# kolinko/effort

Measured on AMD Instinct MI355X. Metric: effective GB/s + tokens/s vs effort %, Mistral-7B FFN 4096x11008 fp16, higher is better.
Workload: dtype f16

## Files before the change

effort_amd/_lib.py:

```python
from __future__ import annotations

import ctypes as C
import os
import subprocess

_HERE = os.path.dirname(os.path.abspath(__file__))
LAB_LIB_PATH = os.path.join(_HERE, "libeffort_hip_lab.so")
LIB_PATH = (LAB_LIB_PATH if os.environ.get("EFFORT_HIP_LIB") == "lab" else os.environ.get("EFFORT_HIP_LIB")) or os.path.join(_HERE, "libeffort_hip.so")

ERRORS = {
    -1: "EFFORT_ERR_ARG", -2: "EFFORT_ERR_SHAPE", -3: "EFFORT_ERR_EFFORT", -4: "EFFORT_ERR_HIP",
    -5: "EFFORT_ERR_KIND", -6: "EFFORT_ERR_CONVERT", -7: "EFFORT_ERR_BLAS", -8: "EFFORT_ERR_COMM",
}


class EffortError(RuntimeError):
    def __init__(self, code: int, where: str, detail: str = ""):
        self.code = code
        super().__init__(f"{where}: {ERRORS.get(code, code)} {detail}".strip())


def build(verbose: bool = False) -> str:
    cmd = ["make", "-C", os.path.join(_HERE, "csrc"), "-j8", "all"]
    res = subprocess.run(cmd, capture_output=not verbose, text=True)
# ... 55 lines not shown
    "effort_convert_status": (C.c_int, [_P, C.POINTER(C.c_int)]),
    "effort_q4_outlier_count": (C.c_int64, [C.c_int, C.c_int, C.c_double]),
    "effort_convert_q4": (C.c_int, [_P, _P, C.c_int, C.c_int, C.c_double, _P, _P, _P, _P]),
    "effort_top2_softmax": (C.c_int, [_P, _P, C.c_int, _P, _P]),
    "effort_mix2": (C.c_int, [_P, _P, _P, _P, _P, C.c_int]),
    "effort_moe_route": (C.c_int, [_P, _P, _P, _P, C.c_int, C.c_int, _P, _P, _P]),
    "effort_mix2_add": (C.c_int, [_P, _P, _P, _P, _P, C.c_int]),
    "effort_dense_gemv": (C.c_int, [_P, _P, _P, _P, C.c_int, C.c_int]),
    "effort_dense_gemv_expert": (C.c_int, [_P, _P, _P, _P, _P, C.c_int, C.c_int, C.c_int]),
    "effort_set_dense_backend": (C.c_int, [_P, C.c_int]),
    "effort_last_dispatch_count": (C.c_int, [_P, C.POINTER(C.c_uint32)]),
    "effort_last_cutoff": (C.c_int, [_P, C.POINTER(C.c_float)]),
    "effort_calc_dispatch": (C.c_int, [_P, _P, _P, _P, C.c_double, _P, _P]),
    "effort_convert_fp16": (C.c_int, [_P, _P, C.c_int, C.c_int, _P, _P, _P]),
    "effort_convert_fp16_pitched": (C.c_int, [_P, _P, C.c_int, C.c_int, _P, C.c_int, _P, _P]),
    "effort_cosine": (C.c_int, [_P, _P, _P, C.c_int, C.POINTER(C.c_float)]),
    "effort_set_split_cutoff": (C.c_int, [_P, C.c_int]),
    "effort_set_tuning": (C.c_int, [_P, C.c_int, C.c_int, C.c_int]),
    "effort_is_lab_build": (C.c_int, []),
    "effort_enable_kernel_timing": (C.c_int, [_P, C.c_int]),
    "effort_debug_stamps": (C.c_int, [_P, C.POINTER(C.c_ulonglong)]),
    "effort_debug_slice_counts": (C.c_int, [_P, C.c_int, C.POINTER(C.c_uint32), C.c_int]),
    "effort_debug_plan": (C.c_int, [C.c_int, C.c_int, C.c_int, C.c_int, _P, _P, _P, _P, _P, _P, C.c_int, C.c_int, C.c_int, C.c_int, _P, _P, _P, _P, _P, _P, _P, _P, _P]),
    "effort_debug_lanes": (C.c_int, [C.c_int, C.c_int, _P, C.c_int64, _P]),
    "effort_debug_trace": (C.c_int, [_P, C.POINTER(C.c_ulonglong), C.c_int]),
    "effort_kernel_clock": (C.c_int, [_P, C.POINTER(C.c_double), C.POINTER(C.c_int)]),
    "effort_kernel_timing": (C.c_int, [_P, C.POINTER(C.c_double), C.POINTER(C.c_double), C.POINTER(C.c_double), C.POINTER(C.c_int)]),
}

_lib = None


def lib() -> C.CDLL:
    global _lib
    if _lib is None:
        if not os.path.exists(LIB_PATH):
            raise RuntimeError(
                f"{LIB_PATH} is missing: the HIP extension has not been built "
                "(run `python -c 'import __graft_entry__ as g; g.build()'` or `make -C effort_amd/csrc`). "
                "effort_amd has no CPU fallback.")
        import torch
        l = C.CDLL(LIB_PATH)
        for name, (res, args) in _SIGS.items():
            if (name.startswith("effort_debug_") or name == "effort_is_lab_build") and os.environ.get("EFFORT_HIP_LIB") and not hasattr(l, name):
                continue
            fn = getattr(l, name)
# ... 9 lines not shown
```

effort_amd/csrc/api.hip:

```cpp
#include <dlfcn.h>
#include <rccl/rccl.h>
#include <rocblas/rocblas.h>

#include <cstdio>
#include <cstring>
#include <map>
#include <mutex>
#include <new>
#include <vector>

#include "../../include/effort_hip.h"
#include "../../include/effort_hip_debug.h"
#include "effort_internal.h"
#include "lanes.h"
#include "plan.h"
#include "sample_device.h"

using namespace effort;

static constexpr size_t kStampBytes = (size_t)(kTraceOff + kTraceItems * 12) * 8;

struct Lane {
    hipStream_t own = nullptr;
    hipEvent_t done = nullptr;
    bool dirty = false;
    float* d_cutoff = nullptr;
    uint32_t* d_count = nullptr;
    float* d_slabs = nullptr;
    uint32_t* d_counters = nullptr;
    uint32_t* d_sliceCounts = nullptr;
    uint32_t* d_queue = nullptr;
    uint32_t lastCalls = 1, lastSliceOff[effort::kMaxGroup] = {0}, lastSlices[effort::kMaxGroup] = {0};
};

struct effort_ctx {
    static constexpr int kMaxLanes = effort::kMaxLanes;
    int device = 0;
    hipStream_t stream = nullptr;
    int numCU = 256;
    Lane lane[kMaxLanes];
    LaneBook book;
    int lastLane = 0;
    hipEvent_t forkEv = nullptr;
    size_t slabBytes = 0;
    uint32_t* d_blockScratch = nullptr;
    uint16_t* d_vhalf = nullptr;
    size_t vhalfElems = 0;
    float* d_cos = nullptr;
    uint16_t* d_convVals = nullptr;
    size_t convElems = 0;
    int* d_status = nullptr;
    int persistent = -1;
    static constexpr uint32_t kMaxTiles = 1024, kMaxSlices = 4096;
    static constexpr size_t kSlabBytes = (size_t)64 << 20;
    unsigned long long* d_tstamp = nullptr;
    double wallClockKHz = 100000.0;
    rocblas_handle blas = nullptr;
    ncclComm_t comm = nullptr;
    int commRank = 0, commWorld = 1;
    bool denseRocblas = false;
    int tuneW = 0, tuneE = 0, tuneS = 0;
    bool splitCutoff = false;
    bool rowReuse = false;
    bool timing = false;
    bool clock = false;
// ... 581 lines not shown
        ga.tstamp = c->clock ? c->d_tstamp : nullptr;
        ga.ablate = env.ablate; ga.trace = (c->clock && c->trace) ? 1u : 0u;
        ga.split = (c->splitCutoff ? 1u : 0u) | (lp.compact ? 4u : 0u) | (c->rowReuse ? 8u : 0u);
        ga.numCU = (uint32_t)c->numCU; ga.queue = L.d_queue;
        ga.count = lp.count; ga.totalTiles = lp.totalTiles; ga.totalItems = lp.totalItems;
        ga.persistent = lp.persistent; ga.cutJobs = lp.cutJobs; ga.staggerSleeps = lp.staggerSleeps;
        for (uint32_t k = 0; k < lp.count; k++) {
            const int i = (int)(lp.first + k);
            const effort_w* w = ws[i];
            const CallPlan& p = plan.call[i];
            CallDesc& a = ga.call[k];
            a.buckets = w->buckets; a.stats = lp.compact ? (const void*)w->means16 : w->stats; a.rankBound = w->rankBound; a.probes = w->probes; a.v = vs[i];
            a.expNo = expNos ? expNos[i] : nullptr; a.out = outs[i];
            a.ol = OutlierIndex{fmt == kQ4 ? w->olBlockPtr : nullptr, w->olEntry, w->olMeta};
            a.q = (uint16_t)(int)((double)(kProbes - 1) * (1.0 - efforts[i]));
            a.bucketsTrim = (uint16_t)w->viewTrim;
            a.pre = pc[i].pre; a.vAux = a.pre ? vAux[i] : nullptr; a.resid = resids ? resids[i] : nullptr;
            a.slabOff = p.slabOff; a.tileOff = (uint16_t)p.tileOff; a.sliceOff = (uint16_t)p.sliceOff; a.geom = (uint16_t)p.geom;
            ga.geom[p.geom] = p.g;
            ga.wgEnd8[k] = (uint16_t)p.itemEnd8;
            L.lastSliceOff[i] = p.sliceOff; L.lastSlices[i] = p.g.slices;
        }
        { const int frc = fork_lane(c, lc); if (frc != EFFORT_OK) return frc; }
        if (c->splitCutoff && !(env.ablate & 1u)) HIP_TRY(c, launch_find_cutoff_group(ga, st));
        HIP_TRY(c, launch_bucket_mul(fmt, plan.W, plan.E, ga, st));
    }
    L.lastCalls = (uint32_t)n;
    if (tm) { HIP_TRY(c, hipEventRecord(ev[1], st)); c->nSamples++; }
    return EFFORT_OK;
}

extern "C" int effort_bucketmul(effort_ctx* c, const effort_w* w, const float* v, const uint32_t* expNo, float* out, double effort) {
    return do_group(c, kFp16, 1, &w, &v, &expNo, &out, &effort);
}
extern "C" int effort_bucketmul_q4(effort_ctx* c, const effort_w* w, const float* v, const uint32_t* expNo, float* out, double effort) {
    return do_group(c, kQ4, 1, &w, &v, &expNo, &out, &effort);
}
extern "C" int effort_bucketmul_group(effort_ctx* c, int n, const effort_w* const* ws, const float* const* vs,
                                      const uint32_t* const* expNos, float* const* outs, const double* efforts) {
    return do_group(c, kFp16, n, ws, vs, expNos, outs, efforts);
}
extern "C" int effort_bucketmul_group_fused(effort_ctx* c, int n, const effort_w* const* ws, const float* const* vs,
                                            const uint32_t* const* expNos, float* const* outs, const double* efforts,
                                            const int* prologues, const void* const* vAux, const float* const* resids) {
    return do_group(c, kFp16, n, ws, vs, expNos, outs, efforts, prologues, vAux, resids);
}
// ... 31 lines not shown
    Lane& L = c->lane[c->lastLane];
    if (L.lastSlices[idx] == 0) {
        HIP_TRY(c, hipMemcpyAsync(host_out, L.d_count, 4, hipMemcpyDeviceToHost, c->stream));
        HIP_TRY(c, hipStreamSynchronize(c->stream));
        return EFFORT_OK;
    }
    static thread_local uint32_t h[effort_ctx::kMaxSlices];
    HIP_TRY(c, hipMemcpyAsync(h, L.d_sliceCounts + L.lastSliceOff[idx], (size_t)L.lastSlices[idx] * 4, hipMemcpyDeviceToHost, c->stream));
    HIP_TRY(c, hipStreamSynchronize(c->stream));
    uint32_t n = 0;
    for (uint32_t i = 0; i < L.lastSlices[idx]; i++) n += h[i];
    *host_out = n;
    return EFFORT_OK;
}
extern "C" int effort_debug_slice_counts(effort_ctx* c, int idx, uint32_t* host, int maxSlices) {
    if (!c || !host || idx < 0 || (uint32_t)idx >= c->lane[c->lastLane].lastCalls || maxSlices < 1) return EFFORT_ERR_ARG;
    { const int jrc = join_lanes(c); if (jrc != EFFORT_OK) return jrc; }
    Lane& L = c->lane[c->lastLane];
    const uint32_t n = L.lastSlices[idx] < (uint32_t)maxSlices ? L.lastSlices[idx] : (uint32_t)maxSlices;
    if (n) HIP_TRY(c, hipMemcpyAsync(host, L.d_sliceCounts + L.lastSliceOff[idx], (size_t)n * 4, hipMemcpyDeviceToHost, c->stream));
    HIP_TRY(c, hipStreamSynchronize(c->stream));
    return (int)n;
}
extern "C" int effort_debug_plan(int q4, int numCU, int lanes, int n, const int* inDim, const int* outDim, const int* percentLoad,
                                 const int* prologue, const int* hasResid, const double* effort, int persistent, int tuneW, int tuneE, int tuneS,
                                 int* we, int* slices, int* tiles, int* sliceRows, int* launchOf,
                                 int* launchPersistent, int* launchCutJobs, int* launchCompact, int* launchStagger) {
    if (numCU < 1 || lanes < 1 || lanes > effort_ctx::kMaxLanes || n < 1 || n > kMaxGroup || !inDim || !outDim || !effort || !we || !slices || !tiles ||
        !sliceRows || !launchOf || !launchPersistent || !launchCutJobs || !launchCompact || !launchStagger) return EFFORT_ERR_ARG;
    const Format fmt = q4 ? kQ4 : kFp16;
    effort_ctx c0;
    c0.numCU = numCU; c0.book.nLanes = lanes; c0.persistent = persistent; c0.tuneW = tuneW; c0.tuneE = tuneE; c0.tuneS = tuneS;
    c0.slabBytes = effort_ctx::kSlabBytes;
    PlanCall pc[kMaxGroup];
    for (int i = 0; i < n; i++) {
        const int load = q4 ? 8 : (percentLoad ? percentLoad[i] : 16);
        if (inDim[i] <= 0 || outDim[i] <= 0 || check_shape((uint32_t)inDim[i], (uint32_t)outDim[i]) != EFFORT_OK || load < 1 || load > 16) return EFFORT_ERR_SHAPE;
        if (!(effort[i] >= 0.0 && effort[i] <= 1.0)) return EFFORT_ERR_EFFORT;
        const uint32_t cols = (uint32_t)outDim[i] / (q4 ? 32u : 16u);
        pc[i] = PlanCall{(uint32_t)inDim[i], (uint32_t)outDim[i], cols, (uint32_t)load, cols * 2u, 1u, !q4, (uint16_t)(prologue ? prologue[i] : 0), hasResid && hasResid[i]};
    }
    GroupPlan plan;
    const int rc = plan_group(fmt, plan_env(&c0, lanes > 1, thin_effort(n, effort)), n, pc, &plan);
    if (rc != EFFORT_OK) return rc;
    we[0] = plan.W; we[1] = plan.E;
    for (int i = 0; i < n; i++) {
        const CallPlan& p = plan.call[i];
        slices[i] = (int)p.g.slices; tiles[i] = (int)p.g.tiles; sliceRows[i] = (int)p.g.sliceRows; launchOf[i] = (int)p.launch;
    }
    for (uint32_t l = 0; l < plan.nLaunches; l++) {
        const LaunchPlan& lp = plan.launch[l];
        launchPersistent[l] = (int)lp.persistent; launchCutJobs[l] = (int)lp.cutJobs; launchCompact[l] = lp.compact ? 1 : 0; launchStagger[l] = (int)lp.staggerSleeps;
    }
    return (int)plan.nLaunches;
}
extern "C" int effort_group_cutoff(effort_ctx* c, int idx, float* host_out) {
    if (!c || !host_out || idx < 0 || (uint32_t)idx >= c->lane[c->lastLane].lastCalls) return EFFORT_ERR_ARG;
    { const int jrc = join_lanes(c); if (jrc != EFFORT_OK) return jrc; }
    Lane& L = c->lane[c->lastLane];
    HIP_TRY(c, hipMemcpyAsync(host_out, L.d_cutoff + idx, 4, hipMemcpyDeviceToHost, c->stream));
    HIP_TRY(c, hipStreamSynchronize(c->stream));
    return EFFORT_OK;
}
extern "C" int effort_last_dispatch_count(effort_ctx* c, uint32_t* host_out) { return effort_group_dispatch_count(c, 0, host_out); }
extern "C" int effort_last_cutoff(effort_ctx* c, float* host_out) { return effort_group_cutoff(c, 0, host_out); }

extern "C" int effort_set_dense_backend(effort_ctx* c, int rocblas) {
    if (!c) return EFFORT_ERR_ARG;
    c->denseRocblas = rocblas != 0;
    return EFFORT_OK;
}
extern "C" int effort_dense_gemv(effort_ctx* c, const void* W, const float* v, float* out, int inDim, int outDim) {
    if (!c || !W || !v || !out || inDim <= 0 || outDim <= 0) return fail(c, EFFORT_ERR_ARG, "dense_gemv: bad argument");
    { const int jrc = join_lanes(c); if (jrc != EFFORT_OK) return jrc; }
    if (inDim % 16) return fail(c, EFFORT_ERR_SHAPE, "dense_gemv: inDim % 16 != 0 (helpers/mps.swift:18)");
    if (!c->denseRocblas && dense_gemv_supported((uint32_t)inDim, (uint32_t)outDim)) {
        HIP_TRY(c, launch_dense_gemv(static_cast<const uint16_t*>(W), v, out, (uint32_t)inDim, (uint32_t)outDim, c->stream));
        return EFFORT_OK;
// ... 301 lines not shown
```

effort_amd/csrc/bucket_mul.hip:

```cpp
#include <cstring>
#include <type_traits>

#include "cutoff_device.h"

namespace effort {

constexpr int kBatch = 16;
template <int E> __host__ __device__ constexpr int batch_rows() { return E >= 4 ? 8 : kBatch; }
constexpr int kRounds = 16;

#ifndef EFFORT_ABLATE_NOSCATTER
#define EFFORT_ABLATE_NOSCATTER 0
#endif
#ifndef EFFORT_ABLATE_NOLOAD
#define EFFORT_ABLATE_NOLOAD 0
#endif

constexpr int kMinWavesPerEU = 4;

#ifndef EFFORT_ROW_AUX
#define EFFORT_ROW_AUX 2
#endif
constexpr int kRowAux = EFFORT_ROW_AUX;
#define GA_PERSISTENT(ga) (PERSIST ? (ga).persistent : 0u)
// ... 163 lines not shown
        }
    } else
#pragma unroll
    for (int rr = 0; rr < kRounds; rr++) {
        if ((uint32_t)(rr * NT) + wave * 64u >= nSlots) continue;
        const uint32_t c = rr * NT + tid;
        uint32_t voff;
        if (FMT == kFp16) {
            const uint32_t rank = c >> lg, jl = c & mask;
            const bool ok = rank < rowsPerIn && jl < nb;
            voff = (rowBase + (ok ? rank * inDim + j0 + jl : j0)) * 8u + 4u;
        } else {
            voff = ((rowBase + j0 * 8u + (c < nSlots ? c : 0u)) * 2u + 1u) * 4u;
        }
        lds_dma_dword(rs, voff, ldsM + ((uint32_t)(rr * NT) + wave * 64u) * 4u);
    }
#pragma unroll
    for (int u = 0; u < (FMT == kFp16 ? 1 : 2); u++) {
        if ((uint32_t)(u * NT) + wave * 64u >= nb) continue;
        lds_dma_dword(rv, (j0 + (uint32_t)(u * NT + tid)) * 4u, ldsV + ((uint32_t)(u * NT) + wave * 64u) * 4u);
    }
}

template <int FMT, int E, int W, bool FUSED, bool COMPACT, bool PERSIST, typename Prefetch>
__device__ __forceinline__ void mul_item(const GroupKArgs& ga, const uint32_t item, const ItemRef& ref, char* smem, const LdsPlan& lp, uint32_t& cachedCall,
                                         float& cachedCutoff, const uint32_t par, const bool staged, const bool firstItem, Prefetch prefetch) {
    constexpr int NACC = Fmt<FMT>::kAcc;
    constexpr int TILE_F = NACC * E * 64;
    constexpr int TILE_L = Fmt<FMT>::kSlots * E * 64;
    constexpr int NT = 64 * W;
    constexpr int VPT = 4096 / NT;
    constexpr int KB = batch_rows<E>();

    const uint32_t ci = __builtin_amdgcn_readfirstlane(ref.ci), s = __builtin_amdgcn_readfirstlane(ref.s), t = __builtin_amdgcn_readfirstlane(ref.t);
    const CallDesc& a = ga.call[ci];
    const MulGeom& g = ga.geom[a.geom];
    float* const a_slabs = ga.slabs + (size_t)a.slabOff * 64u;
    uint32_t* const a_counters = ga.counters + a.tileOff;
    uint32_t* const a_sliceCounts = ga.sliceCounts + a.sliceOff;
    float* const a_cutoff = ga.cutoff + ci;
    (void)item;

    int tid0 = threadIdx.x;
    asm volatile("" : "+v"(tid0));
    const int tid = tid0, lane = tid & 63;
#ifdef EFFORT_CUT_FINE
    const bool wstamp = false;
#else
    const bool wstamp = GA_TSTAMP(ga) && tid == 0;
#endif
    unsigned long long ph[6] = {0, 0, 0, 0, 0, 0};
    if (wstamp) ph[0] = wall_clock64();
#ifdef EFFORT_CUT_FINE
    const bool stampCut = GA_TSTAMP(ga) && item == 0 && tid == 0, stamp = false;
#define EFFORT_PSTAMP(i) if (stampCut) GA_TSTAMP(ga)[26 + (i)] = clock64();
#else
#define EFFORT_PSTAMP(i)
// ... 286 lines not shown
            before[rr] = wtot;
            const uint32_t c = rr * NT + tid;
            bool k;
            if (FMT == kFp16) k = (cutoff < (kCutoffScale * half_bits_to_float((uint16_t)(mraw[u] >> 16))) * ax) & ((c >> lg) < g.rowsPerIn) & sel;
            else k = (cutoff < (kCutoffScale * __uint_as_float(mraw[u])) * fabsf(vq[u])) & (c < nSlots) & sel;
            keepMask |= k ? (1u << rr) : 0u;
            wtot += (uint32_t)__popcll(__ballot(k));
        }
    }
    uint32_t wbase = 0;
    if (lane == 0) wbase = atomicAdd(&flags[4], wtot);
    wbase = __builtin_amdgcn_readfirstlane(wbase);
#pragma unroll
    for (int rr = 0; rr < kRounds; rr++) {
        if ((uint32_t)(rr * NT) >= nSlots) break;
        const uint32_t c = rr * NT + tid;
        const bool k = (keepMask >> rr) & 1u;
        const unsigned long long m = __ballot(k);
        const uint32_t pos = wbase + before[rr] + __builtin_amdgcn_mbcnt_hi((uint32_t)(m >> 32), __builtin_amdgcn_mbcnt_lo((uint32_t)m, 0u));
        if (k) list[pos] = (uint16_t)(FMT == kFp16 ? (((c >> lg) << 12) | (c & ((1u << lg) - 1u))) : c);
    }
    __syncthreads();
    const uint32_t n = flags[4];
    const uint32_t code0 = list[(uint32_t)(wave * KB) + ((uint32_t)lane & (uint32_t)(KB - 1))];
    if (t == 0 && tid == 0) a_sliceCounts[s] = n;
    if (stamp) GA_TSTAMP(ga)[19] = wall_clock64();
    if (wstamp) ph[3] = wall_clock64();

    if constexpr (PERSIST) stream_geom();
    const bool colOK = vColOK != 0u;
    const __amdgpu_buffer_rsrc_t rsrc = __builtin_amdgcn_make_buffer_rsrc(
        reinterpret_cast<uint16_t*>((size_t)(uint32_t)__builtin_amdgcn_readfirstlane(vBuckLo) | ((size_t)(uint32_t)__builtin_amdgcn_readfirstlane(vBuckHi) << 32)), 0,
        (int)__builtin_amdgcn_readfirstlane(vRecords), 0x00020000);
    const uint32_t nU = (GA_ABLATE(ga) & 4u) ? 0u : __builtin_amdgcn_readfirstlane(n);
    uint32_t* const cursor = flags + 5;
    auto grab = [&]() -> uint32_t {
        uint32_t bq = 0;
        if (lane == 0) bq = atomicAdd(cursor, (uint32_t)KB);
        return __builtin_amdgcn_readfirstlane(bq);
    };

    auto decode_code = [&](uint32_t code, uint32_t& boff, float& dv) {
        {
            uint32_t rowIdx;
            if (FMT == kFp16) { const uint32_t rank = code >> 12, jl = code & 4095u; rowIdx = rank * vInDim + jl; dv = vblk[jl] * scale; }
            else {
                rowIdx = code;
                dv = __int_as_float(__float2int_rn((vblk[code >> 3] * means[code]) * scale));
            }
            boff = (vRow0 + rowIdx) * vRowPitch;
        }
    };
    auto decode = [&](uint32_t i0, uint32_t& boff, float& dv) {
// ... 119 lines not shown
            accumulate(pa, dvA, __builtin_amdgcn_readfirstlane(min((uint32_t)KB, nU - baseA)));
            if constexpr (OL) ol_add(entA);
            baseA = grab();
            decode(baseA, boffA, dvA);
            issue(aux, pa, boffA);
            if constexpr (OL) ol_fetch(entA);
            accumulate(pb, dvB, __builtin_amdgcn_readfirstlane(baseB < nU ? min((uint32_t)KB, nU - baseB) : 0u));
            if constexpr (OL) ol_add(entB);
        }
        if constexpr (OL) {
            while (olKa < olK1) {
                ol_fetch(entB); ol_add(entA);
                if (olKa >= olK1) break;
                ol_fetch(entA); ol_add(entB);
            }
        }
    };
    constexpr bool kRowSwitch = kRowAux != 0 && (PERSIST || E == 4);
    const bool rowsReused = kRowSwitch && (ga.split & 8u) != 0u;
    auto stream = [&](auto withOl) {
        if constexpr (kRowSwitch) { if (rowsReused) { stream_rows(withOl, std::integral_constant<int, 0>{}); return; } }
        stream_rows(withOl, std::integral_constant<int, kRowAux>{});
    };
    if constexpr (kOlMerge) { if (olEarly) stream(std::true_type{}); else stream(std::false_type{}); }
    else stream(std::false_type{});
    if (!asked) asked = prefetch();
    __syncthreads();
    if (stamp) GA_TSTAMP(ga)[20] = wall_clock64();
    if (wstamp) ph[4] = wall_clock64();

    float* const olsum = reinterpret_cast<float*>(smem + offM);
    if constexpr (FMT != kFp16) {
        if (olAny) {
            const OutlierIndex& ol = a.ol;
            float* const vfull = olEarly ? reinterpret_cast<float*>(smem + __builtin_amdgcn_readfirstlane(lp.offO)) : olsum + (olPer > kOlSumFloats ? olPer : kOlSumFloats);
            const bool vLds = g.inDim <= kOlLdsFloats;
            if constexpr (!kOlMerge) ol_share();
            const uint32_t bFirst = olBFirst, nB = olNB, parts = olParts;
            if (vLds && !olEarly) {
                for (uint32_t i0 = 0; i0 < g.inDim; i0 += NT * 8u) {
                    float x[8];
#pragma unroll
                    for (int u = 0; u < 8; u++) x[u] = a.v[min(i0 + u * NT + tid, g.inDim - 1u)];
                    if constexpr (FUSED) {
                        uint32_t xa[8];
#pragma unroll
// ... 123 lines not shown
            rec[1] = (unsigned long long)(__builtin_amdgcn_s_getreg((31 << 11) | 20) & 0xFu) | ((unsigned long long)(ci & 0xFu) << 4) | ((unsigned long long)(n & 0xFFFFu) << 8) | ((unsigned long long)(t & 0xFFu) << 24) |
                     ((unsigned long long)__builtin_amdgcn_s_getreg((31 << 11) | 4) << 32);
#pragma unroll
            for (int i = 0; i < 6; i++) rec[2 + i] = ph[i];
        }
        unsigned long long* line = GA_TSTAMP(ga) + 64 + (item & 31u) * 8u;
#pragma unroll
        for (int i = 0; i < 5; i++) atomicAdd(&line[i], ph[i + 1] - ph[i]);
        atomicAdd(&line[5], 1ull);
        atomicMin(&GA_TSTAMP(ga)[0], ph[0]);
        atomicMax(&GA_TSTAMP(ga)[26], ph[0]);
        atomicMax(&GA_TSTAMP(ga)[28], ph[5] - ph[0]);
        atomicMax(&GA_TSTAMP(ga)[29], ph[4] - ph[3]);
        atomicMax(&GA_TSTAMP(ga)[1], (unsigned long long)wall_clock64());
#endif
    };
    {
        __syncthreads();
        if (tid == 0) {
            const uint32_t ticket = __hip_atomic_fetch_add(&a_counters[t], 1u, __ATOMIC_RELAXED, __HIP_MEMORY_SCOPE_AGENT);
            flags[0] = (ticket == nSlices - 1u) ? 1u : 0u;
        }
        __syncthreads();
        if (flags[0] == 0u) { flush_stamps(); return; }
    }
    if (GA_ABLATE(ga) & 2u) { if (tid == 0) __hip_atomic_store(&a_counters[t], 0u, __ATOMIC_RELAXED, __HIP_MEMORY_SCOPE_AGENT); return; }

    const bool rstamp = GA_TSTAMP(ga) && ci == 0 && t == 0 && tid == 0;
    if (rstamp) GA_TSTAMP(ga)[23] = wall_clock64();
    typedef uint32_t u4v __attribute__((ext_vector_type(4)));
    const uint32_t sliceStride = __builtin_amdgcn_readfirstlane(vSliceStride);
    constexpr int kCols4 = TILE_F / 4;
    constexpr int G = NT / kCols4 >= 2 ? NT / kCols4 : 1;
    float* const gpart = reinterpret_cast<float*>(smem + offA + (uint32_t)TILE_L * 4u);
    static_assert(G == 1 || (uint32_t)TILE_L * 4u + (uint32_t)G * TILE_F * 4u <= (cutoff_table_bytes(NT) > (uint32_t)TILE_L * 4u ? cutoff_table_bytes(NT) : (uint32_t)TILE_L * 4u),
                  "the thread groups' partial sums must fit behind the tile");
    auto reduce_tile = [&](auto kc) {
        constexpr int kRed = decltype(kc)::value;
        const int grp = G > 1 ? tid / kCols4 : 0;
        const uint32_t per = G > 1 ? ((nSlices + G - 1) / G + 3u) / 4u * 4u : nSlices;
        const uint32_t sl0 = (uint32_t)grp * per, sl1 = min(nSlices, sl0 + per);
        for (int o = (G > 1 ? tid % kCols4 : tid) * 4; o < TILE_F; o += (G > 1 ? kCols4 : NT) * 4) {
            const uint32_t vo = t * (uint32_t)(TILE_F * 4) + (uint32_t)o * 4u;
            float res[4] = {0.0f, 0.0f, 0.0f, 0.0f};
            if (FUSED && a.resid && (G == 1 || grp == 0)) {
#pragma unroll
                for (int h = 0; h < 4; h++) {
// ... 48 lines not shown
    if (nSlices <= 8u * G) reduce_tile(std::integral_constant<int, 8>{});
    else reduce_tile(std::integral_constant<int, 16>{});
    if (PERSIST && G > 1) __syncthreads();
    if (rstamp) GA_TSTAMP(ga)[24] = wall_clock64();
    if (tid == 0) {
        __hip_atomic_store(&a_counters[t], 0u, __ATOMIC_RELAXED, __HIP_MEMORY_SCOPE_AGENT);
#if !defined(EFFORT_CUT_FINE) && !defined(EFFORT_PRODUCT_ONLY)
        if (GA_TSTAMP(ga)) {
            flush_stamps();
            const uint32_t done = __hip_atomic_fetch_add(ga.groupDone, 1u, __ATOMIC_RELAXED, __HIP_MEMORY_SCOPE_AGENT);
            if (done == ga.totalTiles - 1u) {
                const unsigned long long t0 = __hip_atomic_load(&GA_TSTAMP(ga)[0], __ATOMIC_RELAXED, __HIP_MEMORY_SCOPE_AGENT);
                const unsigned long long t1 = __hip_atomic_load(&GA_TSTAMP(ga)[1], __ATOMIC_RELAXED, __HIP_MEMORY_SCOPE_AGENT);
                GA_TSTAMP(ga)[2] += t1 - t0; GA_TSTAMP(ga)[3] += 1;
                GA_TSTAMP(ga)[27] += __hip_atomic_load(&GA_TSTAMP(ga)[26], __ATOMIC_RELAXED, __HIP_MEMORY_SCOPE_AGENT) - t0;
                __hip_atomic_store(&GA_TSTAMP(ga)[26], 0ull, __ATOMIC_RELAXED, __HIP_MEMORY_SCOPE_AGENT);
                __hip_atomic_store(&GA_TSTAMP(ga)[0], ~0ull, __ATOMIC_RELAXED, __HIP_MEMORY_SCOPE_AGENT);
                __hip_atomic_store(&GA_TSTAMP(ga)[1], 0ull, __ATOMIC_RELAXED, __HIP_MEMORY_SCOPE_AGENT);
                __hip_atomic_store(ga.groupDone, 0u, __ATOMIC_RELAXED, __HIP_MEMORY_SCOPE_AGENT);
            }
        }
#endif
    }
}

template <int NT>
__device__ __forceinline__ void cutoff_job(const GroupKArgs& ga, uint32_t ci, char* smem) {
    constexpr int VPT = 4096 / NT;
    const CallDesc& a = ga.call[ci];
    int tid0 = threadIdx.x;
    asm volatile("" : "+v"(tid0));
    const int tid = tid0;
    const uint32_t e = a.expNo ? a.expNo[0] : 0u;
    const uint16_t* pr = a.probes + (size_t)e * kProbes;
    float vj[VPT]; uint16_t prj[VPT];
#pragma unroll
    for (int i = 0; i < VPT; i++) { vj[i] = a.v[tid + NT * i]; prj[i] = pr[tid + NT * i]; }
    [[maybe_unused]] constexpr bool PERSIST = true;
    const unsigned long long tj0 = (GA_TSTAMP(ga) && GA_TRACE(ga)) ? wall_clock64() : 0ull;
    const float cutoff = block_find_cutoff<NT>(vj, prj, a.q, smem + cutoff_table_bytes(NT), reinterpret_cast<uint32_t*>(smem), []() {}, nullptr);
    if (tid == 0 && GA_TSTAMP(ga) && GA_TRACE(ga)) {
        unsigned long long* rec = GA_TSTAMP(ga) + kTraceOff + (size_t)ci * 8u;
        rec[0] = (unsigned long long)ci | ((unsigned long long)blockIdx.x << 32) | (1ull << 63);
        rec[1] = (unsigned long long)__builtin_amdgcn_s_getreg((31 << 11) | 20) | ((unsigned long long)__builtin_amdgcn_s_getreg((31 << 11) | 4) << 32);
        rec[2] = tj0; rec[3] = wall_clock64();
    }
// ... 11 lines not shown
    __shared__ unsigned long long s_next;
#ifdef EFFORT_CUT_FINE
    if (GA_TSTAMP(ga) && blockIdx.x == 0 && threadIdx.x == 0) GA_TSTAMP(ga)[26] = clock64();
#endif
    if constexpr (!PERSIST) {
        const uint32_t* const kw = reinterpret_cast<const uint32_t*>(&ga);
        uint32_t touch[12];
#pragma unroll
        for (int i = 0; i < 12; i++) touch[i] = kw[i * 16];
#pragma unroll
        for (int i = 0; i < 12; i++) asm volatile("" :: "s"(touch[i]));
    }
#ifdef EFFORT_CUT_FINE
#define EFFORT_ESTAMP(i) if (GA_TSTAMP(ga) && blockIdx.x == 0 && threadIdx.x == 0) GA_TSTAMP(ga)[16 + (i)] = clock64();
#else
#define EFFORT_ESTAMP(i)
#endif
    EFFORT_ESTAMP(0)
    const uint32_t staggerSleeps = ga.staggerSleeps;
    if constexpr (PERSIST) {
        if (GA_PERSISTENT(ga) && staggerSleeps && blockIdx.x >= ga.numCU)
            for (uint32_t i = 0; i < staggerSleeps; i++) __builtin_amdgcn_s_sleep(32);
    }
    const uint32_t total = ga.totalItems + GA_CUTJOBS(ga);
    uint32_t cachedCall = 0xFFFFFFFFu; float cachedCutoff = 0.0f;
    const uint32_t x = blockIdx.x & 7u;
    uint32_t dry = 0;
    auto pull = [&]() -> uint32_t {
        uint32_t got = total;
        for (uint32_t tries = 0; tries < 8u && got >= total; tries++) {
            const uint32_t q = (x + tries) & 7u;
            if ((dry >> q) & 1u) continue;
            const uint32_t cand = __hip_atomic_fetch_add(&ga.queue[q * 16u], 1u, __ATOMIC_RELAXED, __HIP_MEMORY_SCOPE_AGENT) * 8u + q;
            if (cand < total) got = cand; else dry |= 1u << q;
            if (GA_ABLATE(ga) & 64u) break;
        }
        return got;
    };
    auto pull_sync = [&]() -> uint32_t {
        if (threadIdx.x == 0) s_item = pull();
        __syncthreads();
        const uint32_t it = __builtin_amdgcn_readfirstlane(s_item);
        __syncthreads();
        return it;
    };
    constexpr bool kPipe = !FUSED && FMT == kFp16;
    const LdsPlan lp = ga.lp;
    uint32_t par = 0;
    bool staged = false;
    uint32_t gen = 0;
    if (threadIdx.x == 0) __hip_atomic_store(&s_next, 0ull, __ATOMIC_RELAXED, __HIP_MEMORY_SCOPE_WORKGROUP);
    uint32_t item = GA_PERSISTENT(ga) ? pull_sync() : blockIdx.x;
    while (item < total) {
        if (item < GA_CUTJOBS(ga)) {
            if (item < ga.count) cutoff_job<64 * W>(ga, item, smem);
            item = GA_PERSISTENT(ga) ? pull_sync() : total;
            continue;
        }
        ItemRef ref;
        EFFORT_ESTAMP(1)
        if (!locate_item(ga, item - GA_CUTJOBS(ga), ref)) {
            item = GA_PERSISTENT(ga) ? pull_sync() : total;
            continue;
        }
        EFFORT_ESTAMP(2)
        gen++;
        bool stagedNext = false;
        auto prefetch = [&]() -> bool {
            if (!GA_PERSISTENT(ga)) return true;
            if (threadIdx.x == 0)
                __hip_atomic_store(&s_next, ((unsigned long long)gen << 32) | (unsigned long long)pull(), __ATOMIC_RELAXED, __HIP_MEMORY_SCOPE_WORKGROUP);
            const unsigned long long nx = __hip_atomic_load(&s_next, __ATOMIC_RELAXED, __HIP_MEMORY_SCOPE_WORKGROUP);
            if (__builtin_amdgcn_readfirstlane((uint32_t)(nx >> 32)) != gen) return false;
            const uint32_t next = __builtin_amdgcn_readfirstlane((uint32_t)nx);
            ItemRef nref;
            if (kPipe && !(GA_ABLATE(ga) & 128u) && next >= GA_CUTJOBS(ga) && next < total && locate_item(ga, next - GA_CUTJOBS(ga), nref)) {
                int tid0 = threadIdx.x;
                asm volatile("" : "+v"(tid0));
                stage_issue<FMT, W, COMPACT>(ga, nref, tid0, smem, lp, par ^ 1u);
                stagedNext = true;
            }
            return true;
        };
        const bool firstOwn = gen == 1u && (GA_ABLATE(ga) & 512u) != 0u;
        mul_item<FMT, E, W, FUSED, COMPACT, PERSIST>(ga, item - GA_CUTJOBS(ga), ref, smem, lp, cachedCall, cachedCutoff, par, staged, firstOwn, prefetch);
        item = GA_PERSISTENT(ga) ? __builtin_amdgcn_readfirstlane((uint32_t)__hip_atomic_load(&s_next, __ATOMIC_RELAXED, __HIP_MEMORY_SCOPE_WORKGROUP)) : total;
        staged = stagedNext;
        par ^= 1u;
    }
    if (GA_PERSISTENT(ga) && threadIdx.x == 0) {
        const uint32_t gone = __hip_atomic_fetch_add(&ga.queue[8 * 16], 1u, __ATOMIC_RELAXED, __HIP_MEMORY_SCOPE_AGENT);
        if (gone == gridDim.x - 1u) {
            for (int i = 0; i <= 8; i++) __hip_atomic_store(&ga.queue[i * 16], 0u, __ATOMIC_RELAXED, __HIP_MEMORY_SCOPE_AGENT);
            for (int i = 0; i < kMaxGroup; i++) __hip_atomic_store(&ga.queue[9 * 16 + i], 0u, __ATOMIC_RELAXED, __HIP_MEMORY_SCOPE_AGENT);
        }
    }
}

template <int FMT, int E, int W, typename F>
static hipError_t each_variant(F&& f) {
    hipError_t err = hipSuccess;
    auto one = [&](auto fu, auto co, auto pe) {
        constexpr bool FU = decltype(fu)::value, CO = decltype(co)::value, PE = decltype(pe)::value;
        if (err == hipSuccess) err = f(&bucket_mul_kernel<FMT, E, W, FU, CO, PE>, FU, CO, PE);
    };
    constexpr std::true_type T{}; constexpr std::false_type N{};
    one(N, N, T); one(T, N, T);
    if constexpr (FMT == kFp16) one(N, T, T);
// ... 101 lines not shown
```

effort_amd/csrc/plan.h:

```cpp
#pragma once
#include "effort_internal.h"

namespace effort {

constexpr int kMaxLaunches = kMaxGroup / kMaxGeoms + 1;

struct PlanEnv {
    int numCU = 256, nLanes = 1;
    bool laned = false;
    int persistent = -1;
    int tuneW = 0, tuneE = 0, tuneS = 0;
    bool splitCutoff = false, clock = false;
    uint32_t ablate = 0;
    bool noJobs = false, noCompact = false;
    size_t slabBytes = 0;
    uint32_t maxTiles = 0, maxSlices = 0;
    bool thinEffort = false;
    int tailCalls = 0, tailMult = 0;
};
struct PlanCall {
    uint32_t inDim, outDim, cols, rowsPerIn, rowPitch, numExperts;
    bool hasMeans16;
    uint16_t pre;
    bool hasResid;
};
struct CallPlan {
    MulGeom g;
    uint32_t mult;
    uint32_t launch, geom;
    uint32_t slabOff, tileOff, sliceOff;
    uint32_t itemEnd8;
};
struct LaunchPlan {
    uint32_t first, count;
    uint32_t persistent, cutJobs, staggerSleeps;
    bool compact;
    uint32_t totalItems, totalTiles, realItems;
};
struct GroupPlan {
    int W = 0, E = 0;
    int err = 0;
    const char* msg = "";
    uint32_t nLaunches = 0;
    CallPlan call[kMaxGroup];
    LaunchPlan launch[kMaxLaunches];
};

bool supported(int W, int E);
int plan_group(Format fmt, const PlanEnv& env, int n, const PlanCall* calls, GroupPlan* plan);

}
```

effort_amd/csrc/plan.hip:

```cpp
#include <cstring>

#include "../../include/effort_hip.h"
#include "plan.h"

namespace effort {

static uint32_t round8(uint32_t x) { return (x + 7u) / 8u * 8u; }
static uint32_t min_slices(uint32_t inDim) { return round8((inDim + 511u) / 512u); }
static uint32_t max_slices(uint32_t inDim) { return round8((inDim + 127u) / 128u); }
static uint32_t tiles_at(const PlanCall& w, int E) { return (w.cols + 64 * E - 1) / (64 * E); }
static uint32_t group_tiles(int n, const PlanCall* ws, int E) {
    uint32_t t = 0;
    for (int i = 0; i < n; i++) t += tiles_at(ws[i], E);
    return t;
}
static uint32_t padded_items(uint32_t tiles, uint32_t slices) { return round8(tiles * slices); }
static uint32_t padded_min_items(int n, const PlanCall* ws, int E) {
    uint32_t t = 0;
    for (int i = 0; i < n; i++) t += padded_items(tiles_at(ws[i], E), min_slices(ws[i].inDim));
    return t;
}
static bool fits_one_round(const PlanEnv& env, int n, uint32_t tiles, uint32_t allTiles, uint32_t s) {
    const bool same = allTiles == (uint32_t)n * tiles;
    return (same ? (uint32_t)n * padded_items(tiles, s) : allTiles * s + 7u * (uint32_t)n) <= (uint32_t)env.numCU;
// ... 153 lines not shown
static uint32_t geom_index(MulGeom* geoms, uint32_t& n, const MulGeom& g) {
    uint32_t k = 0;
    while (k < n && memcmp(&geoms[k], &g, sizeof(g)) != 0) k++;
    if (k == n && n < (uint32_t)kMaxGeoms) geoms[n++] = g;
    return k;
}

static void finish_launch(Format fmt, const PlanEnv& env, int W, const PlanCall* ws, const GroupPlan* P, LaunchPlan* lp) {
    const uint32_t R = env.persistent < 0 ? 2u : (uint32_t)env.persistent;
    const uint32_t perCU = (env.persistent < 0 && fmt == kFp16 && !env.laned) ? 6u : R;
    lp->persistent = (R && lp->realItems > (uint32_t)env.numCU * perCU) ? R : 0u;
    bool plain = true;
    for (uint32_t i = 0; i < lp->count; i++) plain = plain && !ws[lp->first + i].pre;
    lp->cutJobs = (lp->persistent && !env.splitCutoff && plain && !env.noJobs) ? (lp->count + 7u) / 8u * 8u : 0u;
    const bool leanGrid = lp->persistent == 0u && W == 8 && !env.clock && !env.ablate;
    bool compact = fmt == kFp16 && !env.noCompact && (leanGrid || (lp->persistent != 0u && plain));
    for (uint32_t i = 0; compact && !leanGrid && i < lp->count; i++) compact = !ws[lp->first + i].hasResid;
    for (uint32_t i = 0; compact && i < lp->count; i++) {
        const MulGeom& g = P->call[lp->first + i].g;
        compact = ws[lp->first + i].hasMeans16 && g.inDim % 2u == 0u && g.sliceRows % 2u == 0u;
    }
    lp->compact = compact;
    lp->staggerSleeps = (lp->persistent && fmt == kQ4 && !env.laned) ? 11u : 0u;
}

int plan_group(Format fmt, const PlanEnv& env, int n, const PlanCall* ws, GroupPlan* P) {
    P->err = EFFORT_OK; P->msg = ""; P->nLaunches = 0;
    const bool laned = env.laned;
    const int W = env.tuneW ? env.tuneW : 8;
    const int E = pick_elems(env, fmt, n, ws);
    P->W = W; P->E = E;
    const char* const noGeometry = "bucketmul: no launch geometry for this shape/tuning";
    if (!supported(W, E)) return plan_fail(P, EFFORT_ERR_ARG, noGeometry);
    const uint32_t groupTiles = group_tiles(n, ws, E);
    MulGeom g1[kMaxGroup], g2[kMaxGroup];
    uint32_t it1[kMaxGroup], base = 0;
    for (int i = 0; i < n; i++) {
        const int rc = choose_geom(env, fmt, ws[i], n, W, E, groupTiles, 1, &g1[i]);
        if (rc != EFFORT_OK) return plan_fail(P, rc, noGeometry);
        it1[i] = padded_items(g1[i].tiles, g1[i].slices);
        base += it1[i];
    }
    int thinFrom = n;
    if (E == 2 && n >= 8 && !laned && !env.tuneS && env.persistent < 0 && !env.thinEffort) {
        const uint32_t round = 2u * (uint32_t)env.numCU, over = base % round;
        if (base > round && over != 0u && over * 32u <= round * 7u && (fmt != kFp16 || base <= 6u * (uint32_t)env.numCU)) {
// ... 65 lines not shown
```

effort_amd/runtime.py:

```python
from __future__ import annotations

import ctypes as C

import torch

from . import _lib


class Gpu:
    def __init__(self, device: int | None = None):
        if not torch.cuda.is_available():
            raise RuntimeError("effort_amd needs an AMD GPU (torch.cuda.is_available() is False); there is no CPU fallback")
        self.device = torch.cuda.current_device() if device is None else int(device)
        self._lib = _lib.lib()
        with torch.cuda.device(self.device):
            stream = torch.cuda.current_stream(self.device).cuda_stream
            self.ctx = self._lib.effort_create(self.device, C.c_void_p(stream))
        self.has_comm = False
        self.dense_rocblas = False
        if not self.ctx:
            raise RuntimeError("effort_create failed: " + (self._lib.effort_last_error(None) or b"").decode())
        self._stream = stream

    def _bind_stream(self):
# ... 105 lines not shown
            self.check(k, "slice_counts")
        return list(buf[:k])

    def debug_trace(self, n: int = 4096):
        buf = (C.c_ulonglong * (12 * n))()
        self.check(self._lib.effort_debug_trace(self.ctx, buf, n), "debug_trace")
        return [tuple(buf[8 * i:8 * i + 8]) + tuple(buf[8 * n + 4 * i:8 * n + 4 * i + 4]) for i in range(n)]

    def kernel_timing(self):
        mul, cut, integ, n = C.c_double(), C.c_double(), C.c_double(), C.c_int()
        self.check(self._lib.effort_kernel_timing(self.ctx, C.byref(mul), C.byref(cut), C.byref(integ), C.byref(n)), "kernel_timing")
        return {"mul_us": mul.value, "cutoff_us": cut.value, "integrate_us": integ.value, "samples": n.value}

    def last_dispatch_count(self, idx: int = 0) -> int:
        n = C.c_uint32()
        self.check(self._lib.effort_group_dispatch_count(self.ctx, int(idx), C.byref(n)), "last_dispatch_count")
        return int(n.value)

    def last_cutoff(self, idx: int = 0) -> float:
        x = C.c_float()
        self.check(self._lib.effort_group_cutoff(self.ctx, int(idx), C.byref(x)), "last_cutoff")
        return float(x.value)

    def close(self):
        if getattr(self, "ctx", None):
            self._lib.effort_destroy(self.ctx)
            self.ctx = None

    def __del__(self):
        try:
            self.close()
        except Exception:
            pass


def plan(calls, *, q4: bool = False, numCU: int = 256, lanes: int = 1, persistent: int = -1, waves: int = 0, elems: int = 0, slices: int = 0) -> dict:
    n = len(calls)
    rows = [tuple(c) + (16, 0, 0)[len(c) - 3:] for c in calls]
    ints = lambda k: (C.c_int * n)(*[int(r[k]) for r in rows])
    out = [(C.c_int * max(n, 2))() for _ in range(9)]
    k = _lib.lib().effort_debug_plan(int(q4), numCU, lanes, n, ints(0), ints(1), ints(3), ints(4), ints(5), (C.c_double * n)(*[float(r[2]) for r in rows]),
                                     persistent, waves, elems, slices, *out)
    if k < 0:
        raise _lib.EffortError(k, "plan")
    we, per_call, per_launch = out[0], out[1:5], out[5:]
    res = {"W": we[0], "E": we[1]}
    res.update({name: list(a[:n]) for name, a in zip(("slices", "tiles", "sliceRows", "launch"), per_call)})
    res.update({name: list(a[:k]) for name, a in zip(("persistent", "cutJobs", "compact", "stagger"), per_launch)})
    return res


def lanes(ops, *, lanes: int = 4) -> list[dict]:
    kinds = {"launch": 0, "timed": 1, "join": 2}
    words = []
    for op in ops:
        kind, cap, busy, rd, wr = tuple(op) + (0, (), ())[len(op) - 2:]
        words += [kinds[kind], int(cap), int(bool(busy)), len(rd), len(wr)]
        for lo, hi in list(rd) + list(wr):
            words += [int(lo), int(hi)]
    n, W = len(ops), 18
    out = (C.c_int64 * max(n * W, 1))()
    k = _lib.lib().effort_debug_lanes(lanes, n, (C.c_int64 * max(len(words), 1))(*words), len(words), out)
    if k < 0:
        raise _lib.EffortError(k, "lanes")
    members = lambda mask: tuple(i for i in range(lanes) if mask >> i & 1)
    res = []
    for i in range(n):
        r = out[i * W:(i + 1) * W]
        res.append({"rc": r[0], "joined_first": bool(r[1]), "joined": members(r[2]), "lane": r[3], "fork_waited": bool(r[4]), "waits": members(r[5]),
                    "pending": members(r[6]), "nextLane": r[7], "busyStreak": r[8], "migrated": bool(r[9]),
                    "reads": list(r[10:10 + lanes]), "writes": list(r[14:14 + lanes])})
    return res
# ... 14 lines not shown
```

include/effort_hip_debug.h:

```cpp
#ifndef EFFORT_HIP_DEBUG_H
#define EFFORT_HIP_DEBUG_H

#include "effort_hip.h"

#ifdef __cplusplus
extern "C" {
#endif

EFFORT_API int effort_set_tuning(effort_ctx* ctx, int wavesPerGroup, int elemsPerLane, int rowSlices);
EFFORT_API int effort_set_split_cutoff(effort_ctx* ctx, int split);

EFFORT_API int effort_set_persistent(effort_ctx* ctx, int wgPerCU);

EFFORT_API int effort_debug_hook_lane(effort_ctx* ctx, int lane);

EFFORT_API int effort_is_lab_build(void);
EFFORT_API int effort_enable_kernel_timing(effort_ctx* ctx, int enable);
EFFORT_API int effort_kernel_clock(effort_ctx* ctx, double* mul_us_avg, int* n_launches);
EFFORT_API int effort_kernel_timing(effort_ctx* ctx, double* mul_us_avg, double* cutoff_us_avg,
                         double* integrate_us_avg, int* n_samples);
EFFORT_API int effort_debug_occupancy(effort_ctx* ctx, int q4, int waves, int elems, int ldsBytes);
EFFORT_API int effort_debug_stamps(effort_ctx* ctx, unsigned long long* host32);
EFFORT_API int effort_debug_slice_counts(effort_ctx* ctx, int idx, uint32_t* host, int maxSlices);
EFFORT_API int effort_debug_plan(int q4, int numCU, int lanes, int n, const int* inDim, const int* outDim, const int* percentLoad,
                      const int* prologue, const int* hasResid, const double* effort, int persistent, int tuneW, int tuneE, int tuneS,
                      int* we, int* slices, int* tiles, int* sliceRows, int* launchOf,
                      int* launchPersistent, int* launchCutJobs, int* launchCompact, int* launchStagger);
#define EFFORT_LANES_LAUNCH 0
#define EFFORT_LANES_TIMED 1
#define EFFORT_LANES_JOIN 2
#define EFFORT_LANES_OUT_WORDS 18
EFFORT_API int effort_debug_lanes(int lanes, int nOps, const int64_t* ops, int64_t nWords, int64_t* out);
EFFORT_API int effort_debug_trace(effort_ctx* ctx, unsigned long long* host, int maxRecords);

#ifdef __cplusplus
}
#endif
#endif
```

Before: 21490.

## Let persistent fp16 workgroups walk all tiles of a slice when lanes overlap

Adds a 'walk' mode for persistent compact fp16 launches. When other lanes are pending, each work unit is a (call, slice) pair, and the workgroup loops over every tile of that slice itself instead of pulling per-tile items. Slices are rotated per call to spread load. This is meant to cut work-queue traffic and per-item setup when the GPU is shared across concurrent lanes, at the cost of coarser load balancing and a more complex kernel loop. Debug entry points expose the unit count.

```diff
diff --git a/effort_amd/_lib.py b/effort_amd/_lib.py
--- a/effort_amd/_lib.py
+++ b/effort_amd/_lib.py
@@ -101,6 +101,8 @@
     "effort_debug_stamps": (C.c_int, [_P, C.POINTER(C.c_ulonglong)]),
     "effort_debug_slice_counts": (C.c_int, [_P, C.c_int, C.POINTER(C.c_uint32), C.c_int]),
     "effort_debug_plan": (C.c_int, [C.c_int, C.c_int, C.c_int, C.c_int, _P, _P, _P, _P, _P, _P, C.c_int, C.c_int, C.c_int, C.c_int, _P, _P, _P, _P, _P, _P, _P, _P, _P]),
+    "effort_debug_last_units": (C.c_int, [_P]),
+    "effort_debug_walk_units": (C.c_int, [C.c_int, C.c_int, C.c_int, C.c_int, _P, _P, _P, _P, _P, _P, C.c_int, C.c_int, C.c_int, C.c_int, C.c_int]),
     "effort_debug_lanes": (C.c_int, [C.c_int, C.c_int, _P, C.c_int64, _P]),
     "effort_debug_trace": (C.c_int, [_P, C.POINTER(C.c_ulonglong), C.c_int]),
     "effort_kernel_clock": (C.c_int, [_P, C.POINTER(C.c_double), C.POINTER(C.c_int)]),
diff --git a/effort_amd/csrc/api.hip b/effort_amd/csrc/api.hip
--- a/effort_amd/csrc/api.hip
+++ b/effort_amd/csrc/api.hip
@@ -41,6 +41,7 @@
     Lane lane[kMaxLanes];
     LaneBook book;
     int lastLane = 0;
+    uint32_t lastUnits = 0;
     hipEvent_t forkEv = nullptr;
     size_t slabBytes = 0;
     uint32_t* d_blockScratch = nullptr;
@@ -668,6 +669,8 @@
             L.lastSliceOff[i] = p.sliceOff; L.lastSlices[i] = p.g.slices;
         }
         { const int frc = fork_lane(c, lc); if (frc != EFFORT_OK) return frc; }
+        c->lastUnits = walk_units(plan, l, lc.laned, (c->book.pending_lanes() & ~(1u << lc.pick.lane)) != 0u);
+        if (c->lastUnits) ga.split |= 16u | (c->lastUnits / 8u) << 8;
         if (c->splitCutoff && !(env.ablate & 1u)) HIP_TRY(c, launch_find_cutoff_group(ga, st));
         HIP_TRY(c, launch_bucket_mul(fmt, plan.W, plan.E, ga, st));
     }
@@ -745,12 +748,9 @@
     HIP_TRY(c, hipStreamSynchronize(c->stream));
     return (int)n;
 }
-extern "C" int effort_debug_plan(int q4, int numCU, int lanes, int n, const int* inDim, const int* outDim, const int* percentLoad,
-                                 const int* prologue, const int* hasResid, const double* effort, int persistent, int tuneW, int tuneE, int tuneS,
-                                 int* we, int* slices, int* tiles, int* sliceRows, int* launchOf,
-                                 int* launchPersistent, int* launchCutJobs, int* launchCompact, int* launchStagger) {
-    if (numCU < 1 || lanes < 1 || lanes > effort_ctx::kMaxLanes || n < 1 || n > kMaxGroup || !inDim || !outDim || !effort || !we || !slices || !tiles ||
-        !sliceRows || !launchOf || !launchPersistent || !launchCutJobs || !launchCompact || !launchStagger) return EFFORT_ERR_ARG;
+static int debug_plan_group(int q4, int numCU, int lanes, int n, const int* inDim, const int* outDim, const int* percentLoad, const int* prologue,
+                            const int* hasResid, const double* effort, int persistent, int tuneW, int tuneE, int tuneS, GroupPlan& plan) {
+    if (numCU < 1 || lanes < 1 || lanes > effort_ctx::kMaxLanes || n < 1 || n > kMaxGroup || !inDim || !outDim || !effort) return EFFORT_ERR_ARG;
     const Format fmt = q4 ? kQ4 : kFp16;
     effort_ctx c0;
     c0.numCU = numCU; c0.book.nLanes = lanes; c0.persistent = persistent; c0.tuneW = tuneW; c0.tuneE = tuneE; c0.tuneS = tuneS;
@@ -763,8 +763,15 @@
         const uint32_t cols = (uint32_t)outDim[i] / (q4 ? 32u : 16u);
         pc[i] = PlanCall{(uint32_t)inDim[i], (uint32_t)outDim[i], cols, (uint32_t)load, cols * 2u, 1u, !q4, (uint16_t)(prologue ? prologue[i] : 0), hasResid && hasResid[i]};
     }
+    return plan_group(fmt, plan_env(&c0, lanes > 1, thin_effort(n, effort)), n, pc, &plan);
+}
+extern "C" int effort_debug_plan(int q4, int numCU, int lanes, int n, const int* inDim, const int* outDim, const int* percentLoad,
+                                 const int* prologue, const int* hasResid, const double* effort, int persistent, int tuneW, int tuneE, int tuneS,
+                                 int* we, int* slices, int* tiles, int* sliceRows, int* launchOf,
+                                 int* launchPersistent, int* launchCutJobs, int* launchCompact, int* launchStagger) {
+    if (!we || !slices || !tiles || !sliceRows || !launchOf || !launchPersistent || !launchCutJobs || !launchCompact || !launchStagger) return EFFORT_ERR_ARG;
     GroupPlan plan;
-    const int rc = plan_group(fmt, plan_env(&c0, lanes > 1, thin_effort(n, effort)), n, pc, &plan);
+    const int rc = debug_plan_group(q4, numCU, lanes, n, inDim, outDim, percentLoad, prologue, hasResid, effort, persistent, tuneW, tuneE, tuneS, plan);
     if (rc != EFFORT_OK) return rc;
     we[0] = plan.W; we[1] = plan.E;
     for (int i = 0; i < n; i++) {
@@ -777,6 +784,15 @@
     }
     return (int)plan.nLaunches;
 }
+extern "C" int effort_debug_walk_units(int q4, int numCU, int lanes, int n, const int* inDim, const int* outDim, const int* percentLoad,
+                                       const int* prologue, const int* hasResid, const double* effort, int persistent, int tuneW, int tuneE, int tuneS,
+                                       int othersPending) {
+    GroupPlan plan;
+    const int rc = debug_plan_group(q4, numCU, lanes, n, inDim, outDim, percentLoad, prologue, hasResid, effort, persistent, tuneW, tuneE, tuneS, plan);
+    if (rc != EFFORT_OK) return rc;
+    return (int)walk_units(plan, 0, lanes > 1, othersPending != 0);
+}
+extern "C" int effort_debug_last_units(effort_ctx* c) { return c ? (int)c->lastUnits : EFFORT_ERR_ARG; }
 extern "C" int effort_group_cutoff(effort_ctx* c, int idx, float* host_out) {
     if (!c || !host_out || idx < 0 || (uint32_t)idx >= c->lane[c->lastLane].lastCalls) return EFFORT_ERR_ARG;
     { const int jrc = join_lanes(c); if (jrc != EFFORT_OK) return jrc; }
diff --git a/effort_amd/csrc/bucket_mul.hip b/effort_amd/csrc/bucket_mul.hip
--- a/effort_amd/csrc/bucket_mul.hip
+++ b/effort_amd/csrc/bucket_mul.hip
@@ -209,9 +209,14 @@
     }
 }
 
+template <int FMT, int E, int W, bool FUSED, bool COMPACT, bool PERSIST>
+constexpr bool walk_built() {
+    return PERSIST && COMPACT && !FUSED && FMT == kFp16 && W >= 8 && W < 8 * E;
+}
 template <int FMT, int E, int W, bool FUSED, bool COMPACT, bool PERSIST, typename Prefetch>
 __device__ __forceinline__ void mul_item(const GroupKArgs& ga, const uint32_t item, const ItemRef& ref, char* smem, const LdsPlan& lp, uint32_t& cachedCall,
-                                         float& cachedCutoff, const uint32_t par, const bool staged, const bool firstItem, Prefetch prefetch) {
+                                         float& cachedCutoff, const uint32_t par, const bool staged, const bool firstItem, const bool walk, Prefetch prefetch) {
+    constexpr bool kWalk = walk_built<FMT, E, W, FUSED, COMPACT, PERSIST>();
     constexpr int NACC = Fmt<FMT>::kAcc;
     constexpr int TILE_F = NACC * E * 64;
     constexpr int TILE_L = Fmt<FMT>::kSlots * E * 64;
@@ -219,7 +224,8 @@
     constexpr int VPT = 4096 / NT;
     constexpr int KB = batch_rows<E>();
 
-    const uint32_t ci = __builtin_amdgcn_readfirstlane(ref.ci), s = __builtin_amdgcn_readfirstlane(ref.s), t = __builtin_amdgcn_readfirstlane(ref.t);
+    const uint32_t ci = __builtin_amdgcn_readfirstlane(ref.ci), s = __builtin_amdgcn_readfirstlane(ref.s);
+    uint32_t t = __builtin_amdgcn_readfirstlane(ref.t);
     const CallDesc& a = ga.call[ci];
     const MulGeom& g = ga.geom[a.geom];
     float* const a_slabs = ga.slabs + (size_t)a.slabOff * 64u;
@@ -552,13 +558,13 @@
     }
     __syncthreads();
     const uint32_t n = flags[4];
-    const uint32_t code0 = list[(uint32_t)(wave * KB) + ((uint32_t)lane & (uint32_t)(KB - 1))];
+    uint32_t code0 = list[(uint32_t)(wave * KB) + ((uint32_t)lane & (uint32_t)(KB - 1))];
     if (t == 0 && tid == 0) a_sliceCounts[s] = n;
     if (stamp) GA_TSTAMP(ga)[19] = wall_clock64();
     if (wstamp) ph[3] = wall_clock64();
 
     if constexpr (PERSIST) stream_geom();
-    const bool colOK = vColOK != 0u;
+    bool colOK = vColOK != 0u;
     const __amdgpu_buffer_rsrc_t rsrc = __builtin_amdgcn_make_buffer_rsrc(
         reinterpret_cast<uint16_t*>((size_t)(uint32_t)__builtin_amdgcn_readfirstlane(vBuckLo) | ((size_t)(uint32_t)__builtin_amdgcn_readfirstlane(vBuckHi) << 32)), 0,
         (int)__builtin_amdgcn_readfirstlane(vRecords), 0x00020000);
@@ -724,6 +730,21 @@
         if constexpr (kRowSwitch) { if (rowsReused) { stream_rows(withOl, std::integral_constant<int, 0>{}); return; } }
         stream_rows(withOl, std::integral_constant<int, kRowAux>{});
     };
+    const uint32_t tEnd = (kWalk && walk) ? g.tiles : t + 1u;
+    bool again = false;
+    for (;;) {
+    if constexpr (kWalk) {
+        if (again) {
+            for (int i = tid; i < TILE_L; i += NT) acc[i] = 0;
+            if (tid == 0) *cursor = (uint32_t)(W * KB);
+            code0 = list[(uint32_t)(wave * KB) + ((uint32_t)lane & (uint32_t)(KB - 1))];
+            stream_geom();
+            colOK = vColOK != 0u;
+            vSlabOff += (uint32_t)(TILE_F * 4);
+            __syncthreads();
+        }
+        asked = t + 1u < tEnd;
+    }
     if constexpr (kOlMerge) { if (olEarly) stream(std::true_type{}); else stream(std::false_type{}); }
     else stream(std::false_type{});
     if (!asked) asked = prefetch();
@@ -893,7 +914,12 @@
             flags[0] = (ticket == nSlices - 1u) ? 1u : 0u;
         }
         __syncthreads();
-        if (flags[0] == 0u) { flush_stamps(); return; }
+        if (flags[0] == 0u) {
+            flush_stamps();
+            if (!kWalk || t + 1u >= tEnd) return;
+            t++; again = true;
+            continue;
+        }
     }
     if (GA_ABLATE(ga) & 2u) { if (tid == 0) __hip_atomic_store(&a_counters[t], 0u, __ATOMIC_RELAXED, __HIP_MEMORY_SCOPE_AGENT); return; }
 
@@ -988,6 +1014,9 @@
         }
 #endif
     }
+    if (!kWalk || t + 1u >= tEnd) break;
+    t++; again = true;
+    }
 }
 
 template <int NT>
@@ -1045,7 +1074,19 @@
         if (GA_PERSISTENT(ga) && staggerSleeps && blockIdx.x >= ga.numCU)
             for (uint32_t i = 0; i < staggerSleeps; i++) __builtin_amdgcn_s_sleep(32);
     }
-    const uint32_t total = ga.totalItems + GA_CUTJOBS(ga);
+    constexpr bool kWalk = walk_built<FMT, E, W, FUSED, COMPACT, PERSIST>();
+    const bool walk = kWalk && (ga.split & 16u) != 0u;
+    const uint32_t total = (walk ? (ga.split >> 8) * 8u : ga.totalItems) + GA_CUTJOBS(ga);
+    auto locate = [&](const uint32_t idx, ItemRef& r) -> bool {
+        if constexpr (kWalk) {
+            if (walk) {
+                const uint32_t S = ga.geom[0].slices, ci = __builtin_amdgcn_readfirstlane(idx / S), b = idx - ci * S;
+                r.ci = ci; r.s = (b >> 3) * 8u + (((b & 7u) + ci) & 7u); r.t = 0u;
+                return true;
+            }
+        }
+        return locate_item(ga, idx, r);
+    };
     uint32_t cachedCall = 0xFFFFFFFFu; float cachedCutoff = 0.0f;
     const uint32_t x = blockIdx.x & 7u;
     uint32_t dry = 0;
@@ -1082,7 +1123,7 @@
         }
         ItemRef ref;
         EFFORT_ESTAMP(1)
-        if (!locate_item(ga, item - GA_CUTJOBS(ga), ref)) {
+        if (!locate(item - GA_CUTJOBS(ga), ref)) {
             item = GA_PERSISTENT(ga) ? pull_sync() : total;
             continue;
         }
@@ -1097,7 +1138,7 @@
             if (__builtin_amdgcn_readfirstlane((uint32_t)(nx >> 32)) != gen) return false;
             const uint32_t next = __builtin_amdgcn_readfirstlane((uint32_t)nx);
             ItemRef nref;
-            if (kPipe && !(GA_ABLATE(ga) & 128u) && next >= GA_CUTJOBS(ga) && next < total && locate_item(ga, next - GA_CUTJOBS(ga), nref)) {
+            if (kPipe && !(GA_ABLATE(ga) & 128u) && next >= GA_CUTJOBS(ga) && next < total && locate(next - GA_CUTJOBS(ga), nref)) {
                 int tid0 = threadIdx.x;
                 asm volatile("" : "+v"(tid0));
                 stage_issue<FMT, W, COMPACT>(ga, nref, tid0, smem, lp, par ^ 1u);
@@ -1106,7 +1147,7 @@
             return true;
         };
         const bool firstOwn = gen == 1u && (GA_ABLATE(ga) & 512u) != 0u;
-        mul_item<FMT, E, W, FUSED, COMPACT, PERSIST>(ga, item - GA_CUTJOBS(ga), ref, smem, lp, cachedCall, cachedCutoff, par, staged, firstOwn, prefetch);
+        mul_item<FMT, E, W, FUSED, COMPACT, PERSIST>(ga, item - GA_CUTJOBS(ga), ref, smem, lp, cachedCall, cachedCutoff, par, staged, firstOwn, walk, prefetch);
         item = GA_PERSISTENT(ga) ? __builtin_amdgcn_readfirstlane((uint32_t)__hip_atomic_load(&s_next, __ATOMIC_RELAXED, __HIP_MEMORY_SCOPE_WORKGROUP)) : total;
         staged = stagedNext;
         par ^= 1u;
diff --git a/effort_amd/csrc/plan.h b/effort_amd/csrc/plan.h
--- a/effort_amd/csrc/plan.h
+++ b/effort_amd/csrc/plan.h
@@ -35,6 +35,7 @@
     uint32_t first, count;
     uint32_t persistent, cutJobs, staggerSleeps;
     bool compact;
+    bool walk;
     uint32_t totalItems, totalTiles, realItems;
 };
 struct GroupPlan {
@@ -48,5 +49,6 @@
 
 bool supported(int W, int E);
 int plan_group(Format fmt, const PlanEnv& env, int n, const PlanCall* calls, GroupPlan* plan);
+uint32_t walk_units(const GroupPlan& plan, uint32_t l, bool laned, bool othersPending);
 
 }
diff --git a/effort_amd/csrc/plan.hip b/effort_amd/csrc/plan.hip
--- a/effort_amd/csrc/plan.hip
+++ b/effort_amd/csrc/plan.hip
@@ -199,6 +199,16 @@
     }
     lp->compact = compact;
     lp->staggerSleeps = (lp->persistent && fmt == kQ4 && !env.laned) ? 11u : 0u;
+    bool walk = fmt == kFp16 && lp->persistent != 0u && lp->cutJobs != 0u && compact && W >= 8 && W < 8 * P->E && !env.clock && !env.ablate;
+    const MulGeom& g0 = P->call[lp->first].g;
+    for (uint32_t i = 0; walk && i < lp->count; i++) walk = memcmp(&P->call[lp->first + i].g, &g0, sizeof(g0)) == 0;
+    lp->walk = walk && g0.tiles >= 2u && g0.slices % 8u == 0u;
+}
+
+uint32_t walk_units(const GroupPlan& plan, uint32_t l, bool laned, bool othersPending) {
+    const LaunchPlan& lp = plan.launch[l];
+    if (!lp.walk || !laned || !othersPending) return 0u;
+    return lp.totalItems / plan.call[lp.first].g.tiles;
 }
 
 int plan_group(Format fmt, const PlanEnv& env, int n, const PlanCall* ws, GroupPlan* P) {
diff --git a/effort_amd/runtime.py b/effort_amd/runtime.py
--- a/effort_amd/runtime.py
+++ b/effort_amd/runtime.py
@@ -151,6 +151,12 @@
         self.check(self._lib.effort_group_cutoff(self.ctx, int(idx), C.byref(x)), "last_cutoff")
         return float(x.value)
 
+    def last_units(self) -> int:
+        k = int(self._lib.effort_debug_last_units(self.ctx))
+        if k < 0:
+            self.check(k, "last_units")
+        return k
+
     def close(self):
         if getattr(self, "ctx", None):
             self._lib.effort_destroy(self.ctx)
@@ -177,6 +183,18 @@
     res.update({name: list(a[:n]) for name, a in zip(("slices", "tiles", "sliceRows", "launch"), per_call)})
     res.update({name: list(a[:k]) for name, a in zip(("persistent", "cutJobs", "compact", "stagger"), per_launch)})
     return res
+
+
+def walk_units(calls, *, others_pending: bool, q4: bool = False, numCU: int = 256, lanes: int = 1, persistent: int = -1, waves: int = 0, elems: int = 0,
+               slices: int = 0) -> int:
+    n = len(calls)
+    rows = [tuple(c) + (16, 0, 0)[len(c) - 3:] for c in calls]
+    ints = lambda k: (C.c_int * n)(*[int(r[k]) for r in rows])
+    k = _lib.lib().effort_debug_walk_units(int(q4), numCU, lanes, n, ints(0), ints(1), ints(3), ints(4), ints(5), (C.c_double * n)(*[float(r[2]) for r in rows]),
+                                           persistent, waves, elems, slices, int(bool(others_pending)))
+    if k < 0:
+        raise _lib.EffortError(k, "walk_units")
+    return int(k)
 
 
 def lanes(ops, *, lanes: int = 4) -> list[dict]:
diff --git a/include/effort_hip_debug.h b/include/effort_hip_debug.h
--- a/include/effort_hip_debug.h
+++ b/include/effort_hip_debug.h
@@ -26,6 +26,10 @@
                       const int* prologue, const int* hasResid, const double* effort, int persistent, int tuneW, int tuneE, int tuneS,
                       int* we, int* slices, int* tiles, int* sliceRows, int* launchOf,
                       int* launchPersistent, int* launchCutJobs, int* launchCompact, int* launchStagger);
+EFFORT_API int effort_debug_last_units(effort_ctx* ctx);
+EFFORT_API int effort_debug_walk_units(int q4, int numCU, int lanes, int n, const int* inDim, const int* outDim, const int* percentLoad,
+                      const int* prologue, const int* hasResid, const double* effort, int persistent, int tuneW, int tuneE, int tuneS,
+                      int othersPending);
 #define EFFORT_LANES_LAUNCH 0
 #define EFFORT_LANES_TIMED 1
 #define EFFORT_LANES_JOIN 2
```

Result: slower. 15550 (-27.7%).
